# JuliaParallel/DistributedArrays.jl

Hardware: NVIDIA H100
Metric: GB/s for map! and sum on Float32 DArray (higher is better)
Workload: dtype f32

## Files before the change

distributedarrays.jl_b200/_broadcast.py:

```python
from __future__ import annotations

import ctypes as C
import struct
from typing import Callable, List, Optional, Sequence, Tuple

import numpy as np

from builtins import any as builtins_any

from . import _lib
from ._darray import B200Array, DArray, dab_dtype, darray, makelocal
from .layout import shape_of
from .runtime import close_remote_reads, open_remote_reads, runtime

_RANK = {"bool": 0, "i32": 1, "i64": 2, "i128": 3, "f32": 4, "f64": 5}


class _TagTypes(dict):

    def __missing__(self, tag):
        raise _lib.UnsupportedError(_lib.ERR_UNSUPPORTED, f"values of type {tag} have no array element type on the GPU backend "
                                    "(Int128 is served as the value type of mapreduce(f, op, d) only)")


_NPT = _TagTypes({"bool": np.dtype(np.bool_), "i32": np.dtype(np.int32), "i64": np.dtype(np.int64), "f32": np.dtype(np.float32),
                  "f64": np.dtype(np.float64), "c64": np.dtype(np.complex64), "c128": np.dtype(np.complex128)})
_TAG = {v: k for k, v in _NPT.items()}
SLICE_TRACING = [0]
_CT = {"bool": "bool", "i32": "int", "i64": "long long", "i128": "i128", "f32": "float", "f64": "double", "c64": "jl_c64", "c128": "jl_c128"}
_COMP = {"c64": "f32", "c128": "f64"}
_CPLX_OF = {"f32": "c64", "f64": "c128"}


def is_ctag(t: str) -> bool:
    return t in _COMP


def tag_of(dtype) -> str:
    dt = np.dtype(dtype)
    if dt not in _TAG:
        raise _lib.UnsupportedError(_lib.ERR_UNSUPPORTED, f"element type {dt} not served by the GPU backend")
    return _TAG[dt]


def promote(a: str, b: str) -> str:
    if a == b:
        return a
    if is_ctag(a) or is_ctag(b):
        if "i128" in (a, b):
            raise _lib.UnsupportedError(_lib.ERR_UNSUPPORTED, "Int128 values mixed with complex values are not served")
        return _CPLX_OF[promote(_COMP.get(a, a), _COMP.get(b, b))]
    if "f" in a[0] + b[0]:
        fl = [t for t in (a, b) if t[0] == "f"]
        return "f64" if "f64" in fl else "f32"
    return a if _RANK[a] >= _RANK[b] else b

# ... 706 lines not shown


def _localise(rt, a, I, pid) -> LocalArg:
    if isinstance(a, DArray):
        view = _bcview(a.dims, I)
        arr = makelocal(a, view, pid)
        return LocalArg(arr, None, tag_of(a.dtype), temp=arr is not a.chunks.get(pid))
    if isinstance(a, np.ndarray) and a.ndim > 0:
        view = _bcview(a.shape, I)
        sl = a[tuple(slice(lo - 1, hi) for lo, hi in view)]
        return LocalArg(B200Array.from_numpy(rt, sl), None, tag_of(a.dtype), temp=True)
    e = Expr.wrap(a.item() if isinstance(a, np.ndarray) else a)
    return LocalArg(None, e.val, e.jt)


def _remote_args(dest_layout, args) -> List[DArray]:
    return [a for a in args if isinstance(a, DArray) and not (a.layout.pids == dest_layout.pids and a.layout.indices == dest_layout.indices)]


def _broadcast_chunks(dest: DArray, expr: Expr, args) -> DArray:
    rt = dest.rt
    fenced = open_remote_reads(rt, _remote_args(dest.layout, args), "host")
    for pid, out in dest.chunks.items():
        I = dest.layout.localindices(pid)
        largs = [_localise(rt, a, I, pid) for a in args]
        run_local(rt, expr, out, largs)
        for la in largs:
            if la.temp and la.arr is not None:
                la.arr.free()
    close_remote_reads(rt, fenced, "host")
    return dest


def _materialise_views(args):
    from ._darray import SubDArray
    out, temps = [], []
    for a in args:
        if isinstance(a, SubDArray):
            a = a.to_darray()
            temps.append(a)
        out.append(a)
    return out, temps


def broadcast_into(dest: DArray, f: Callable, *args) -> DArray:
    args, _views = _materialise_views(args)
    try:
        return _broadcast_into(dest, f, *args)
    finally:
        for v in _views:
            v.close()


def _broadcast_into(dest: DArray, f: Callable, *args) -> DArray:
    shapes = [a.dims if isinstance(a, DArray) else (a.shape if isinstance(a, np.ndarray) else ()) for a in args]
    for shp in shapes:
        for k, s in enumerate(shp):
            want = dest.dims[k] if k < len(dest.dims) else 1
            if s != 1 and s != want:
                raise _lib.DimensionMismatch(_lib.ERR_DIM_MISMATCH, f"destination axes {dest.dims} are not compatible with source axes {tuple(shp)}")
    expr = trace(f, [_arg_tag(a) for a in args])
    return _broadcast_chunks(dest, expr, args)


def broadcast(f: Callable, *args, rt=None) -> DArray:
    args, _views = _materialise_views(args)
    try:
        return _broadcast(f, *args, rt=rt)
    finally:
        for v in _views:
            v.close()


def _broadcast(f: Callable, *args, rt=None) -> DArray:
    rt = rt or next((a.rt for a in args if isinstance(a, DArray)), None) or runtime()
    shapes = [a.dims if isinstance(a, DArray) else (a.shape if isinstance(a, np.ndarray) else ()) for a in args]
    dims = _bc_shape(shapes)
    expr = trace(f, [_arg_tag(a) for a in args])
    out_dt = _NPT[expr.jt]
    dest = darray(lambda I: B200Array.empty(rt, shape_of(I), out_dt), dims, dtype=out_dt, rt=rt)
    return _broadcast_chunks(dest, expr, args)


def copy(d: DArray) -> DArray:
    from ._darray import similar
    return _broadcast_into(similar(d), lambda x: x, d)


deepcopy = copy


def drandn(dims, procs=None, dist=None, dtype=np.float64, seed: int = 1234, rt=None) -> DArray:
    from ._darray import component_dtype, drand
    dt = np.dtype(dtype)
    if dt.kind == "c":
        ct = component_dtype(dt)
        re = drandn(dims, procs, dist, dtype=ct, seed=seed, rt=rt)
        im = drandn(dims, procs, dist, dtype=ct, seed=seed + 2, rt=rt)
        from ._darray import darray_like
        out = darray_like(lambda I: B200Array.empty(re.rt, shape_of(I), dt), re, dtype=dt)
        _broadcast_into(out, lambda a, b: complex_(0.7071067811865476 * a, 0.7071067811865476 * b), re, im)
        re.close()
        im.close()
        return out
    if dt.kind != "f":
        raise _lib.UnsupportedError(_lib.ERR_UNSUPPORTED, f"drandn of eltype {dt}")
    u1 = drand(dims, procs, dist, dtype=dt, seed=seed, rt=rt)
    u2 = drand(dims, procs, dist, dtype=dt, seed=seed + 1, rt=rt)
# ... 48 lines not shown
```

distributedarrays.jl_b200/_darray.py:

```python
from __future__ import annotations

import ctypes as C
import itertools
import weakref
from typing import Callable, Dict, List, Optional, Sequence, Tuple

import numpy as np

from . import _lib
from .layout import Layout, Range, default_procs, layout_from_chunk_shapes, make_layout, rlen, shape_of, slab_plan
from .runtime import Runtime, close_remote_reads, open_remote_reads, runtime

_DT = {np.dtype(np.float32): _lib.F32, np.dtype(np.float64): _lib.F64, np.dtype(np.int32): _lib.I32,
       np.dtype(np.int64): _lib.I64, np.dtype(np.bool_): _lib.U8,
       np.dtype(np.complex64): _lib.C64, np.dtype(np.complex128): _lib.C128}
_NP = {_lib.F32: np.dtype(np.float32), _lib.F64: np.dtype(np.float64), _lib.I32: np.dtype(np.int32),
       _lib.I64: np.dtype(np.int64), _lib.U8: np.dtype(np.bool_), _lib.C64: np.dtype(np.complex64), _lib.C128: np.dtype(np.complex128)}


def dab_dtype(dt) -> int:
    dt = np.dtype(dt)
    if dt not in _DT:
        raise _lib.UnsupportedError(_lib.ERR_UNSUPPORTED, f"element type {dt} is not served by the GPU backend (no host fallback)")
    return _DT[dt]


def np_dtype(code: int) -> np.dtype:
    return _NP[code]


def is_complex(dt) -> bool:
    return np.dtype(dt).kind == "c"


def component_dtype(dt) -> np.dtype:
    dt = np.dtype(dt)
    return {np.dtype(np.complex64): np.dtype(np.float32), np.dtype(np.complex128): np.dtype(np.float64)}.get(dt, dt)


_allowscalar = [True]


def allowscalar(flag: bool = True):
    _allowscalar[0] = bool(flag)


class B200Array:

    __slots__ = ("rt", "ptr", "shape", "dtype", "_own", "_keep", "_temp")

    def __init__(self, rt: Runtime, ptr: int, shape: Sequence[int], dtype, own: bool = True, keep=None, temp: bool = False):
        self.rt, self.ptr, self.shape, self.dtype = rt, int(ptr), tuple(int(s) for s in shape), np.dtype(dtype)
        self._own, self._keep, self._temp = own, keep, temp

    @classmethod
    def empty(cls, rt: Runtime, shape: Sequence[int], dtype, temp: bool = False) -> "B200Array":
        dtype = np.dtype(dtype)
        n = int(np.prod(shape)) if len(shape) else 1
        ptr = rt.alloc_temp(n * dtype.itemsize) if temp else rt.alloc(n * dtype.itemsize)
        return cls(rt, ptr, shape, dtype, temp=temp)

    @classmethod
    def from_numpy(cls, rt: Runtime, a: np.ndarray) -> "B200Array":
        a = np.asarray(a)
        dab_dtype(a.dtype)
        out = cls.empty(rt, a.shape, a.dtype)
        out.copy_from_host(a)
        return out

    @property
    def size(self) -> int:
        return int(np.prod(self.shape)) if len(self.shape) else 1

    @property
    def nbytes(self) -> int:
        return self.size * self.dtype.itemsize

    @property
    def ndim(self) -> int:
        return len(self.shape)

    def copy_from_host(self, a: np.ndarray, sync: bool = True):
        a = np.asarray(a, dtype=self.dtype)
        if tuple(a.shape) != self.shape:
            raise _lib.DimensionMismatch(_lib.ERR_DIM_MISMATCH, f"host array {a.shape} vs chunk {self.shape}")
        if self.size == 0:
            return
        if not a.flags.f_contiguous:
            if a.ndim == 2 and a.strides[0] == a.itemsize and a.strides[1] > 0:
                _lib.call("dab_h2d_2d", self.rt.ctx, C.c_void_p(self.ptr), a.shape[0] * a.itemsize, C.c_void_p(a.ctypes.data),
                          a.strides[1], a.shape[0] * a.itemsize, a.shape[1])
                if sync:
                    self.rt.sync()
                return
            a = np.asfortranarray(a)
        _lib.call("dab_h2d", self.rt.ctx, C.c_void_p(self.ptr), C.c_void_p(a.ctypes.data), self.nbytes)
        if sync:
            self.rt.sync()

    def to_numpy(self) -> np.ndarray:
        out = np.empty(self.shape, dtype=self.dtype, order="F")
        if self.size:
            _lib.call("dab_d2h", self.rt.ctx, C.c_void_p(out.ctypes.data), C.c_void_p(self.ptr), self.nbytes)
            self.rt.sync()
        return out

    def free(self):
        if self._own and self.ptr:
            if self._temp:
                self.rt.free_temp(self.ptr)
            else:
                self.rt.free(self.ptr)
        self.ptr = 0

    def __repr__(self):
        return f"B200Array({self.dtype}, {self.shape}, ptr=0x{self.ptr:x}, dev={self.rt.device})"


def pinned_empty(rt: Runtime, shape, dtype) -> np.ndarray:
    dtype = np.dtype(dtype)
    n = int(np.prod(shape)) if len(shape) else 1
    p = C.c_void_p()
    _lib.call("dab_host_alloc", rt.ctx, max(1, n * dtype.itemsize), C.byref(p))
    buf = (C.c_char * max(1, n * dtype.itemsize)).from_address(p.value)
    arr = np.frombuffer(buf, dtype=dtype, count=n).reshape(shape, order="F")
# ... 655 lines not shown
```

distributedarrays.jl_b200/_mapreduce.py:

```python
from __future__ import annotations

import builtins
import ctypes as C
import operator
from itertools import accumulate
from typing import Callable, Dict, Optional, Sequence, Tuple

import numpy as np

from . import _lib
from ._broadcast import Expr, broadcast, is_ctag, tag_of, trace, _NPT
from ._darray import B200Array, DArray, component_dtype, dab_dtype, is_complex, np_dtype
from .layout import Layout, ravel, reduction_passes, shape_of, unravel
from .runtime import close_remote_reads, deliver, exchange_stacks, open_remote_reads

_OPS = {"+": _lib.SUM, "add": _lib.SUM, "sum": _lib.SUM, "*": _lib.PROD, "mul": _lib.PROD, "prod": _lib.PROD, "max": _lib.MAX,
        "min": _lib.MIN}
_OPF = {operator.add: _lib.SUM, operator.mul: _lib.PROD, builtins.max: _lib.MAX, builtins.min: _lib.MIN, np.add: _lib.SUM,
        np.multiply: _lib.PROD, np.maximum: _lib.MAX, np.minimum: _lib.MIN}


def _op_code(op) -> int:
    if isinstance(op, str) and op in _OPS:
        return _OPS[op]
    if op in _OPF:
        return _OPF[op]
    raise _lib.UnsupportedError(_lib.ERR_UNSUPPORTED, f"reduction operator {op!r} is not served by a kernel (no host fallback)")


_CMPMAP = {"eq": _lib.MAP_EQ, "ne": _lib.MAP_NE, "lt": _lib.MAP_LT, "le": _lib.MAP_LE, "gt": _lib.MAP_GT, "ge": _lib.MAP_GE}
_FLIP = {"lt": "gt", "le": "ge", "gt": "lt", "ge": "le", "eq": "eq", "ne": "ne"}


def classify_map(f: Optional[Callable], dtype) -> Tuple[Optional[int], Optional[np.ndarray], Optional[Expr]]:
    if f is None:
        return _lib.MAP_ID, None, None
    tag = tag_of(dtype)
    e = trace(f, [tag])
    if e.op == "arg":
        return _lib.MAP_ID, None, e
    if is_ctag(tag):
        if len(e.args) == 1 and e.args[0].op == "arg":
            code = {"abs": _lib.MAP_ABS, "abs2": _lib.MAP_ABS2, "neg": _lib.MAP_NEG, "isnan": _lib.MAP_ISNAN}.get(e.op)
            if code is not None:
                return code, None, e
        return None, None, e
    if e.jt == tag and len(e.args) == 1 and e.args[0].op == "arg":
        code = {"abs": _lib.MAP_ABS, "abs2": _lib.MAP_ABS2, "neg": _lib.MAP_NEG}.get(e.op)
        if code is not None:
            return code, None, e
    if e.op == "mul" and e.jt == tag and builtins.all(a.op == "arg" for a in e.args):
        return _lib.MAP_ABS2, None, e
    if e.op in _CMPMAP:
        l, r = e.args

        def unpromote(side, const):
            if side.op == "convert" and side.args[0].op == "arg" and side.args[0].jt == tag and const.op == "const":
                c = const.val
                if tag == "f32" and const.jt == "f64" and float(np.float32(c)) == c:
                    return side.args[0], Expr("const", (), tag, c)
                if tag in ("i32", "i64") and const.jt in ("i64",) and side.jt == "i64":
                    return side.args[0], Expr("const", (), tag, c) if -2**31 <= c < 2**31 or tag == "i64" else (side, const)
            return side, const

        l, r = unpromote(l, r)
        r, l = unpromote(r, l)
        if l.op == "arg" and r.op == "const" and l.jt == tag:
            return _CMPMAP[e.op], np.asarray(r.val, dtype=np.dtype(dtype)), e
        if r.op == "arg" and l.op == "const" and r.jt == tag:
            return _CMPMAP[_FLIP[e.op]], np.asarray(l.val, dtype=np.dtype(dtype)), e
    if e.op == "isnan" and e.args[0].op == "arg":
        return _lib.MAP_ISNAN, None, e
    return None, None, e


def _result_dtype(dtype, op: int, mapc: int) -> np.dtype:
    out = C.c_int32()
    _lib.check(_lib.lib().dab_reduce_result_dtype(dab_dtype(dtype), op, mapc, C.byref(out)))
    return np.dtype(np.int64) if out.value == _lib.I64 else np_dtype(out.value)




def _gather_slots(d: DArray, launch: Callable[[int, B200Array, int], None]) -> np.ndarray:
    rt = d.rt
    wpr = rt.workers_per_rank
    slots = B200Array.empty(rt, (16 * wpr,), np.uint8, temp=True)
    try:
        for pid, ch in d.chunks.items():
            launch(pid, ch, slots.ptr + 16 * ((pid - 1) % wpr))
        if rt.world > 1:
            allslots = B200Array.empty(rt, (16 * wpr * rt.world,), np.uint8, temp=True)
            _lib.call("dab_allgather", rt.ctx, C.c_void_p(slots.ptr), C.c_void_p(allslots.ptr), 16 * wpr)
            host = allslots.to_numpy()
            allslots.free()
        else:
            host = slots.to_numpy()
    finally:
        rt.sync()
        slots.free()
    return host.view(np.uint8)


def _fold(host: np.ndarray, pids: Sequence[int], rdt: np.dtype, op: int):
    vals = np.empty(len(pids), dtype=rdt)
    for i, pid in enumerate(pids):
        vals[i] = host[16 * (pid - 1):16 * (pid - 1) + rdt.itemsize].view(rdt)[0]
    out = np.zeros(1, dtype=rdt)
    rcode = _lib.I64 if rdt == np.dtype(np.int64) else dab_dtype(rdt)
    _lib.check(_lib.lib().dab_combine_ordered(rcode, op, C.c_void_p(vals.ctypes.data), len(pids), C.c_void_p(out.ctypes.data)))
    return out[0], vals


def _int128(b: bytes) -> int:
    return int.from_bytes(b, "little", signed=True)


def wrap128(v: int) -> int:
    v &= (1 << 128) - 1
    return v - (1 << 128) if v >> 127 else v


def fold128(vals: Sequence[int], op: int) -> int:
    acc = vals[0]
    for v in vals[1:]:
        acc = wrap128(acc + v) if op == _lib.SUM else wrap128(acc * v) if op == _lib.PROD else (max(acc, v) if op == _lib.MAX else min(acc, v))
    return acc


def _check_nonempty(d: DArray, opc: int):
    if opc in (_lib.MAX, _lib.MIN):
        for pid in d.layout.pids:
# ... 45 lines not shown
        if ch.size == 0:
            return _empty_slot(rt, opc, np.dtype(np.int64) if wide else rdt, slot_ptr)
        I = d.layout.localindices(pid)
        largs = [_localise(rt, a, I, pid) for a in args]
        e, largs = split_c128_scalars(expr, largs)
        if len(largs) > 8:
            raise _lib.UnsupportedError(_lib.ERR_UNSUPPORTED, "more than 8 mapreduce arguments (a ComplexF64 scalar counts twice) are not served")
        src = codegen(e).encode()
        n = len(largs)
        dts = (C.c_int32 * n)(*[dab_dtype(NPT[la.tag]) for la in largs])
        ptrs = (C.c_void_p * n)(*[la.arr.ptr if la.arr is not None else None for la in largs])
        scal = (C.c_uint64 * n)()
        for k, la in enumerate(largs):
            if la.arr is None:
                scal[k] = int.from_bytes(np.asarray(la.scalar, dtype=NPT[la.tag]).tobytes().ljust(8, b"\0"), "little")
            elif la.temp:
                temps.append(la.arr)
        _lib.call("dab_mapreduce_expr", rt.ctx, src, val_code, opc_k, ch.size, n, dts, ptrs, scal, C.c_void_p(slot_ptr))

    try:
        host = _gather_slots(d, launch)
    finally:
        for t in temps:
            t.free()
        close_remote_reads(rt, fenced, "host")
    if wide:
        vals = [_int128(host[16 * (pid - 1):16 * pid].tobytes()) for pid in d.layout.pids]
        res = fold128(vals, opc)
        return (res, vals) if return_partials else res
    res, vals = _fold(host, d.layout.pids, rdt, opc if opc != _lib.COUNT else _lib.SUM)
    return (res, vals) if return_partials else res


def _mapreduce_all(f, op, d: DArray, return_partials: bool = False, others: Sequence = ()):
    opc = op if isinstance(op, int) else _op_code(op)
    if others:
        expr = trace(f, [tag_of(d.dtype)] + [_arg_tag_of(a) for a in others])
        return _mapreduce_expr(expr, opc, d, others, return_partials)
    mapc, param, expr = classify_map(f, d.dtype)
    if is_complex(d.dtype) and mapc is not None and not _complex_served(opc, mapc):
        if mapc == _lib.MAP_ID and opc in (_lib.MAX, _lib.MIN):
            raise TypeError(f"MethodError: no method matching isless(::{d.dtype}, ::{d.dtype}) -- complex numbers are not ordered")
        mapc = None
        if expr is None:
            expr = trace(lambda z: z, [tag_of(d.dtype)])
    if mapc is None:
        return _mapreduce_expr(expr, opc, d, (), return_partials)
    _check_nonempty(d, opc)
    rt = d.rt
    pp = C.c_void_p(param.ctypes.data) if param is not None else None
    rdt = _result_dtype(d.dtype, opc, mapc)
    if rt.workers_per_rank == 1 and d.layout.pids == rt.workers() and not return_partials:
        ch = d.chunks[rt.myid()]
        out = np.zeros(2, dtype=np.uint64)
        _lib.call("dab_mapreduce_all", rt.ctx, dab_dtype(d.dtype), opc, mapc, pp, C.c_void_p(ch.ptr), ch.size, C.c_void_p(out.ctypes.data))
        return out.view(np.uint8)[:rdt.itemsize].view(rdt)[0]
    code = dab_dtype(d.dtype)
    host = _gather_slots(d, lambda pid, ch, slot: _lib.call("dab_reduce", rt.ctx, code, opc, mapc, pp, C.c_void_p(ch.ptr), ch.size, C.c_void_p(slot)))
    res, vals = _fold(host, d.layout.pids, rdt, opc)
    return (res, vals) if return_partials else res


def _complex_served(opc: int, mapc: int) -> bool:
    out = C.c_int32()
    return _lib.lib().dab_reduce_result_dtype(_lib.C64, opc, mapc, C.byref(out)) == _lib.OK


def _arg_tag_of(a) -> str:
    from ._broadcast import _arg_tag
    return _arg_tag(a)


def reduce(op, d: DArray, dims=None, init=None):
    return mapreduce(None, op, d, dims=dims, init=init)


def mapreduce(f: Optional[Callable], op, d: DArray, *ds, dims=None, init=None, _partials: bool = False):
    from ._darray import SubDArray
    if isinstance(d, Expr):
        from . import _slices
        if _slices.tracing():
            return _slices.reduce_of_slice(f, op, d, ds, dims, init)
    if isinstance(d, SubDArray):
        tmp = d.to_darray()
        try:
            return mapreduce(f, op, tmp, *ds, dims=dims, init=init, _partials=_partials)
        finally:
            if dims is None:
                tmp.close()
    if dims is None:
        if init is not None:
            raise _lib.UnsupportedError(_lib.ERR_UNSUPPORTED, "mapreduce(f, op, d; init) without dims falls back to scalar iteration in the reference; not served")
        return _mapreduce_all(f, op, d, _partials, ds)
    if ds:
        tmp = broadcast(f, d, *ds)
        try:
            return mapreducedim(None, op, tmp, dims, init)
        finally:
            tmp.close()
    return mapreducedim(f, op, d, dims, init)


def sum(d: DArray, f: Optional[Callable] = None, dims=None):
    return mapreduce(f, "+", d, dims=dims)


def prod(d: DArray, f: Optional[Callable] = None, dims=None):
    return mapreduce(f, "*", d, dims=dims)

# ... 363 lines not shown
```

distributedarrays.jl_b200/csrc/dab_comm.cu:

```cuda
#include <dlfcn.h>
#include <nccl.h>

#include "dab_common.cuh"
#include "dab_scalar_ops.cuh"

namespace {

struct NcclApi {
    void* handle = nullptr;
    ncclResult_t (*GetUniqueId)(ncclUniqueId*) = nullptr;
    ncclResult_t (*CommInitRank)(ncclComm_t*, int, ncclUniqueId, int) = nullptr;
    ncclResult_t (*CommDestroy)(ncclComm_t) = nullptr;
    ncclResult_t (*AllGather)(const void*, void*, size_t, ncclDataType_t, ncclComm_t, cudaStream_t) = nullptr;
    ncclResult_t (*AllReduce)(const void*, void*, size_t, ncclDataType_t, ncclRedOp_t, ncclComm_t, cudaStream_t) = nullptr;
    ncclResult_t (*Send)(const void*, size_t, ncclDataType_t, int, ncclComm_t, cudaStream_t) = nullptr;
    ncclResult_t (*Recv)(void*, size_t, ncclDataType_t, int, ncclComm_t, cudaStream_t) = nullptr;
    ncclResult_t (*GroupStart)() = nullptr;
    ncclResult_t (*GroupEnd)() = nullptr;
    const char* (*GetErrorString)(ncclResult_t) = nullptr;
    const char* (*GetLastError)(ncclComm_t) = nullptr;
    bool ok = false;
    char why[256] = "";
};

NcclApi& nccl() {
    static NcclApi api;
    static bool tried = false;
    if (tried) return api;
    tried = true;
    const char* names[] = {"libnccl.so.2", "libnccl.so", nullptr};
    for (int i = 0; names[i] && !api.handle; ++i) api.handle = dlopen(names[i], RTLD_NOW | RTLD_GLOBAL);
    if (!api.handle) {
        snprintf(api.why, sizeof(api.why), "dlopen(libnccl.so.2) failed: %s", dlerror());
        return api;
    }
#define SYM(field, name)                                                            \
    do {                                                                            \
        *(void**)(&api.field) = dlsym(api.handle, name);                            \
        if (!api.field) {                                                           \
            snprintf(api.why, sizeof(api.why), "libnccl lacks symbol %s", name);    \
            return api;                                                             \
        }                                                                           \
    } while (0)
    SYM(GetUniqueId, "ncclGetUniqueId");
    SYM(CommInitRank, "ncclCommInitRank");
    SYM(CommDestroy, "ncclCommDestroy");
    SYM(AllGather, "ncclAllGather");
    SYM(AllReduce, "ncclAllReduce");
    SYM(Send, "ncclSend");
    SYM(Recv, "ncclRecv");
    SYM(GroupStart, "ncclGroupStart");
    SYM(GroupEnd, "ncclGroupEnd");
    SYM(GetErrorString, "ncclGetErrorString");
#undef SYM
// ... 109 lines not shown
}

int32_t dab_allreduce(dab_ctx* ctx, int32_t dtype, int32_t op, const void* send_dev, void* recv_dev, size_t count) {
    DAB_ENTER(ctx);
    NEED_COMM(ctx);
    ncclDataType_t dt;
    switch (dtype) {
        case DAB_F32: dt = ncclFloat32; break;
        case DAB_F64: dt = ncclFloat64; break;
        case DAB_I32: dt = ncclInt32; break;
        case DAB_I64: dt = ncclInt64; break;
        case DAB_U8: dt = ncclUint8; break;
        default: return dab_fail(ctx, DAB_ERR_ARG, "dab_allreduce: bad dtype %d", dtype);
    }
    ncclRedOp_t ro;
    switch (op) {
        case DAB_SUM: ro = ncclSum; break;
        case DAB_PROD: ro = ncclProd; break;
        case DAB_MAX: ro = ncclMax; break;
        case DAB_MIN: ro = ncclMin; break;
        default: return dab_fail(ctx, DAB_ERR_ARG, "dab_allreduce: bad op %d", op);
    }
    DAB_NCCL(ctx, api.AllReduce(send_dev, recv_dev, count, dt, ro, (ncclComm_t)ctx->comm, ctx->stream));
    ctx->launches++;
    return DAB_OK;
}

int32_t dab_group_start(dab_ctx* ctx) {
    DAB_ENTER(ctx);
    NEED_COMM(ctx);
    DAB_NCCL(ctx, api.GroupStart());
    return DAB_OK;
}
int32_t dab_group_end(dab_ctx* ctx) {
    DAB_ENTER(ctx);
    NEED_COMM(ctx);
    DAB_NCCL(ctx, api.GroupEnd());
    ctx->launches++;
    return DAB_OK;
}
int32_t dab_send(dab_ctx* ctx, const void* send_dev, size_t nbytes, int32_t peer) {
    DAB_ENTER(ctx);
    NEED_COMM(ctx);
    DAB_NCCL(ctx, api.Send(send_dev, nbytes, ncclInt8, peer, (ncclComm_t)ctx->comm, ctx->stream));
    return DAB_OK;
}
int32_t dab_recv(dab_ctx* ctx, void* recv_dev, size_t nbytes, int32_t peer) {
    DAB_ENTER(ctx);
    NEED_COMM(ctx);
    DAB_NCCL(ctx, api.Recv(recv_dev, nbytes, ncclInt8, peer, (ncclComm_t)ctx->comm, ctx->stream));
    return DAB_OK;
}

int32_t dab_mapreduce_all(dab_ctx* ctx, int32_t dtype, int32_t op, int32_t map, const void* map_param, const void* x, size_t n,
                          void* out_host) {
    DAB_ENTER_NOFLUSH(ctx);
    int32_t rdt;
    if (!out_host || op == DAB_EXTREMA || dab_reduce_result_dtype(dtype, op, map, &rdt) != DAB_OK) {
        DAB_FLUSH(ctx);
        DAB_REQUIRE(ctx, out_host, DAB_ERR_ARG, "dab_mapreduce_all: null out");
        if (op == DAB_EXTREMA) return dab_fail(ctx, DAB_ERR_UNSUPPORTED, "dab_mapreduce_all: extrema combines through dab_reduce + dab_allgather");
        return dab_fail(ctx, DAB_ERR_ARG, "bad dtype/op");
    }
    const bool cplx = rdt == DAB_C64 || rdt == DAB_C128;
    if ((ctx->mbox_ranks > 1 || !ctx->comm || ctx->nranks == 1) && n > 0 && !cplx) {
        ctx->fuse_op = op;
        int32_t st = dab_reduce(ctx, dtype, op, map, map_param, x, n, ctx->result_slot);
        ctx->fuse_op = -1;
        if (st != DAB_OK) return st;
        DAB_CUDA(ctx, cudaStreamSynchronize(ctx->stream));
        const volatile unsigned long long* h = (const volatile unsigned long long*)ctx->host_slot;
        if (h[1] != 0) return dab_fail(ctx, DAB_ERR_NCCL, "fused combine timed out waiting for a peer's chunk result (did every rank call?)");
        unsigned long long bits = h[0];
        memset(out_host, 0, 8);
        memcpy(out_host, &bits, dab_dtype_size(rdt));
        return DAB_OK;
    }
    if (cplx && ctx->mbox_ranks > 1 && !ctx->comm) {
        DAB_FLUSH(ctx);
        return dab_fail(ctx, DAB_ERR_UNSUPPORTED, "dab_mapreduce_all: a complex result across %d ranks needs the NCCL communicator "
                        "(the mailbox combine carries 8-byte results)", ctx->mbox_ranks);
    }
    int32_t st = dab_reduce(ctx, dtype, op, map, map_param, x, n, ctx->result_slot);
    if (st != DAB_OK) return st;
    const int P = ctx->comm ? ctx->nranks : 1;
    const void* src = ctx->result_slot;
    if (P > 1) {
        NEED_COMM(ctx);
        DAB_NCCL(ctx, api.AllGather(ctx->result_slot, ctx->gather_slots, 16, ncclInt8, (ncclComm_t)ctx->comm, ctx->stream));
        ctx->launches++;
        src = ctx->gather_slots;
    }
    DAB_CUDA(ctx, cudaMemcpyAsync(ctx->host_slot, src, (size_t)P * 16, cudaMemcpyDeviceToHost, ctx->stream));
    DAB_CUDA(ctx, cudaStreamSynchronize(ctx->stream));
    unsigned char tmp[DAB_MAX_RANKS * 16];
    size_t es = dab_dtype_size(rdt);
    for (int i = 0; i < P; ++i) memcpy(tmp + (size_t)i * es, (const char*)ctx->host_slot + (size_t)i * 16, es);
    unsigned char res[16] = {0};
    st = dab_combine_ordered(rdt, op, tmp, (size_t)P, res);
    if (st != DAB_OK) return dab_fail(ctx, st, "%s", dab_last_error(nullptr));
    memset(out_host, 0, es > 8 ? es : 8);
    memcpy(out_host, res, es);
    return DAB_OK;
}

int32_t dab_mailbox_create(dab_ctx* ctx, void* handle64) {
    DAB_ENTER(ctx);
    DAB_REQUIRE(ctx, handle64, DAB_ERR_ARG, "dab_mailbox_create: null handle");
    if (!ctx->mailbox) {
        DAB_CUDA(ctx, cudaMalloc(&ctx->mailbox, DAB_MBOX_BYTES));
        DAB_CUDA(ctx, cudaMemset(ctx->mailbox, 0, DAB_MBOX_BYTES));
    }
    cudaIpcMemHandle_t h;
    DAB_CUDA(ctx, cudaIpcGetMemHandle(&h, ctx->mailbox));
    memcpy(handle64, &h, 64);
    return DAB_OK;
}

int32_t dab_mailbox_attach(dab_ctx* ctx, const void* handles, int32_t rank, int32_t nranks) {
    DAB_ENTER(ctx);
    DAB_REQUIRE(ctx, handles && nranks >= 1 && nranks <= DAB_MAX_RANKS && rank >= 0 && rank < nranks, DAB_ERR_ARG, "dab_mailbox_attach: bad arguments");
    DAB_REQUIRE(ctx, ctx->mailbox, DAB_ERR_ARG, "dab_mailbox_attach: call dab_mailbox_create first");
    DAB_REQUIRE(ctx, ctx->mbox_ranks == 0, DAB_ERR_ARG, "mailboxes already attached");
// ... 107 lines not shown
```

distributedarrays.jl_b200/csrc/dab_common.cuh:

```cuda
#pragma once
#include <cuda_runtime.h>

#include <cstdint>
#include <cstdio>
#include <cstring>

#include "../../include/dab200.h"

#define DAB_MAX_REDUCE_BLOCKS 262144
#define DAB_SLOT_BYTES 64
#define DAB_MAX_RANKS 64

struct dab_pending_affine {
    int active;
    int32_t dtype;
    void* y;
    const void* x;
    size_t n;
    unsigned char a[8], b[8];
};

struct dab_ctx {
    int device;
    int sm_count;
    cudaStream_t stream;
    void* block_partials;
    unsigned int* counter;
    void* result_slot;
    void* gather_slots;
    void* host_slot;
    void* dim_scratch;
    size_t dim_scratch_bytes;
    uint64_t launches;
    void* comm;
    int rank, nranks;
    void* mailbox;
    void** peer_mbox_dev;
    void* peer_mbox_host[DAB_MAX_RANKS];
    int mbox_ranks;
    unsigned long long mbox_seq;
    unsigned long long barrier_seq;
    int fuse_op;
    struct dab_alloc_cache* cache;
    void* sort_dev;
    size_t sort_dev_bytes;
    void* stage[2];
    cudaEvent_t stage_ev[2];
    void* sort_host;
    unsigned long long sort_epoch;
    void* scan_dev;
    size_t scan_dev_bytes;
    unsigned long long scan_epoch;
    unsigned long long scan_tickets;
    void* scan_scratch;
    size_t scan_scratch_bytes;
    long long opt_combine_timeout_ms;
    int opt_ew_tma;
    dab_pending_affine pending;
    int defer_off;
    char err[512];
};

extern thread_local char dab_tls_err[512];

int32_t dab_fail(dab_ctx* ctx, int32_t status, const char* fmt, ...);
int32_t dab_fail_cuda(dab_ctx* ctx, cudaError_t e, const char* what, const char* file, int line);

#define DAB_CUDA(ctx, call)                                                             \
    do {                                                                                \
        cudaError_t e__ = (call);                                                       \
        if (e__ != cudaSuccess) return dab_fail_cuda((ctx), e__, #call, __FILE__, __LINE__); \
    } while (0)

#define DAB_REQUIRE(ctx, cond, status, ...)                          \
    do {                                                             \
        if (!(cond)) return dab_fail((ctx), (status), __VA_ARGS__);  \
    } while (0)

int32_t dab_flush_pending(dab_ctx* ctx);

#define DAB_FLUSH(ctx)                                    \
    do {                                                  \
        if ((ctx)->pending.active) {                      \
            int32_t st__ = dab_flush_pending(ctx);        \
            if (st__ != DAB_OK) return st__;              \
        }                                                 \
    } while (0)

#define DAB_ENTER(ctx)                                                      \
    do {                                                                    \
        if ((ctx) == nullptr) return dab_fail(nullptr, DAB_ERR_ARG, "null ctx"); \
        DAB_CUDA((ctx), cudaSetDevice((ctx)->device));                      \
        DAB_FLUSH(ctx);                                                     \
// ... 93 lines not shown
```

distributedarrays.jl_b200/csrc/dab_reduce.cu:

```cuda
#include <type_traits>

#include <cmath>

#include "dab_reduce_traits.cuh"

namespace {

struct NoStore {
    template <typename T>
    __device__ __forceinline__ void vec(Pack<T>&, size_t) const {}
    template <typename T>
    __device__ __forceinline__ T scalar(T v, size_t) const { return v; }
};
template <typename T>
struct AffineStore {
    AffineF<T> f;
    T* y;
    int4* yv;
    __device__ __forceinline__ void vec(Pack<T>& p, size_t i) const {
#pragma unroll
        for (int k = 0; k < Pack<T>::N; ++k) p.v[k] = f(p.v[k]);
        st_stream(yv + i, as_int4(p));
    }
    __device__ __forceinline__ T scalar(T v, size_t i) const {
// ... 45 lines not shown
                for (int w = VPT; w > 1; w >>= 1)
#pragma unroll
                    for (int k = 0; k < w / 2; ++k) m[k] = R::tile(m[k], m[k + w / 2]);
                tv[u] = m[0];
            }
#pragma unroll
            for (int w = RD_UNROLL; w > 1; w >>= 1)
#pragma unroll
                for (int k = 0; k < w / 2; ++k) tv[k] = R::tile(tv[k], tv[k + w / 2]);
            acc = R::comb(acc, R::lift(tv[0]));
        } else {
#pragma unroll
            for (int u = 0; u < RD_UNROLL; ++u) {
                Pack<T> p = as_pack<T>(r[u]);
                st.vec(p, base + (size_t)u * RD_THREADS);
                acc = fold_into<R>(acc, p, map);
            }
        }
    }
    if (blockIdx.x == gridDim.x - 1) {
        for (size_t i = ntiles * TILE + threadIdx.x; i < nvec; i += RD_THREADS) {
            Pack<T> p = as_pack<T>(ld_stream(xv + i));
            st.vec(p, i);
            W m = R::pre(map(p.v[0]));
#pragma unroll
            for (int k = 1; k < VPT; ++k) m = R::tile(m, R::pre(map(p.v[k])));
            acc = R::comb(acc, R::lift(m));
        }
        for (size_t i = threadIdx.x; i < head; i += RD_THREADS) acc = R::comb(acc, R::lift(R::pre(map(st.scalar(x[i], i)))));
        for (size_t i = head + nvec * VPT + threadIdx.x; i < n; i += RD_THREADS)
            acc = R::comb(acc, R::lift(R::pre(map(st.scalar(x[i], i)))));
    }
    acc = block_reduce<R>(acc, smem);
    A fin;
    if (!last_cta_out<R>(acc, partials, counter, smem, is_last, fin)) return;
    if (threadIdx.x == 0) {
        if constexpr (std::is_arithmetic<A>::value) {
            Out res;
            if (finalize_mode == 1) res = (Out)(fin == (A)n_for_all);
            else if (finalize_mode == 2) res = (Out)(fin != (A)0);
            else res = (Out)fin;
            memcpy(out, &res, sizeof(Out));
            if (sizeof(Out) < 8) memset((char*)out + sizeof(Out), 0, 8 - sizeof(Out));
            A wide = fin;
            memcpy((char*)out + 8, &wide, sizeof(A));
            if (sizeof(A) < 8) memset((char*)out + 8 + sizeof(A), 0, 8 - sizeof(A));
            if (fc.host_out && fc.nranks <= 1) {
                unsigned long long bits = 0;
                memcpy(&bits, &res, sizeof(Out));
                volatile unsigned long long* h = reinterpret_cast<volatile unsigned long long*>(fc.host_out);
                h[0] = bits;
                h[1] = 0ull;
                __threadfence_system();
            }
        } else if constexpr (is_cplx<Out>::value) {
            using CT = decltype(Out::re);
            const Out res{(CT)fin.re, (CT)fin.im};
            memset(out, 0, 16);
            memcpy(out, &res, sizeof(Out));
        } else {
            memset(out, 0, 16);
            memcpy(out, &fin, sizeof(A));
        }
    }
    if constexpr (!std::is_arithmetic<Out>::value) return;
    else {
    if (fc.nranks <= 1) return;
    __shared__ unsigned long long pay[2];
    __shared__ unsigned long long got[DAB_MAX_RANKS];
    __shared__ int timed_out;
    if (threadIdx.x == 0) {
        memcpy(&pay[0], out, 8);
        memcpy(&pay[1], (char*)out + 8, 8);
        timed_out = 0;
    }
    __syncthreads();
    const size_t bank = (size_t)(fc.seq & 1ull) * DAB_MAX_RANKS * DAB_MBOX_SLOT;
    if (threadIdx.x < (unsigned)fc.nranks) {
        volatile unsigned long long* dst =
            reinterpret_cast<volatile unsigned long long*>((char*)fc.peers[threadIdx.x] + bank + (size_t)fc.rank * DAB_MBOX_SLOT);
        dst[0] = pay[0];
        dst[1] = pay[1];
        __threadfence_system();
        dst[2] = fc.seq;
        volatile unsigned long long* src =
            reinterpret_cast<volatile unsigned long long*>((char*)fc.peers[fc.rank] + bank + (size_t)threadIdx.x * DAB_MBOX_SLOT);
        const unsigned long long t0 = dab_globaltimer_ns();
        unsigned int spins = 0;
        while (src[2] != fc.seq) {
            if ((++spins & 1023u) == 0 && dab_globaltimer_ns() - t0 > fc.timeout_ns) {
                timed_out = 1;
                break;
            }
        }
        __threadfence_system();
        got[threadIdx.x] = src[0];
    }
    __syncthreads();
    if (threadIdx.x == 0) {
        Out a;
        memcpy(&a, &got[0], sizeof(Out));
        for (int j = 1; j < fc.nranks; ++j) {
            Out b;
            memcpy(&b, &got[j], sizeof(Out));
            switch (fc.op) {
                case DAB_SUM: case DAB_COUNT: a = jl::add(a, b); break;
                case DAB_PROD: a = jl::mul(a, b); break;
                case DAB_MAX: a = jl::max(a, b); break;
                case DAB_MIN: a = jl::min(a, b); break;
                case DAB_ALL: a = (Out)(a != (Out)0 && b != (Out)0); break;
                default: a = (Out)(a != (Out)0 || b != (Out)0); break;
            }
        }
        unsigned long long bits = 0;
        memcpy(&bits, &a, sizeof(Out));
        volatile unsigned long long* h = reinterpret_cast<volatile unsigned long long*>(fc.host_out);
        h[0] = bits;
        h[1] = (unsigned long long)timed_out;
        __threadfence_system();
    }
    }
}

template <typename T, typename Map, typename R, typename Out, typename St = NoStore>
int32_t launch_reduce(dab_ctx* ctx, const T* x, size_t n, Map map, void* out, int finalize_mode, St st = St()) {
    const FlatGrid fg = flat_grid(x, n);
    if constexpr (!std::is_same<St, NoStore>::value) st.yv = reinterpret_cast<int4*>(st.y + fg.head);
    FusedComm fc;
    memset(&fc, 0, sizeof(fc));
    if (ctx->fuse_op >= 0 && ctx->mbox_ranks > 1) {
        fc.peers = ctx->peer_mbox_dev;
        fc.host_out = ctx->host_slot;
        fc.seq = ++ctx->mbox_seq;
        fc.timeout_ns = (unsigned long long)ctx->opt_combine_timeout_ms * 1000000ull;
        fc.rank = ctx->rank;
        fc.nranks = ctx->mbox_ranks;
        fc.op = ctx->fuse_op;
    } else if (ctx->fuse_op >= 0) {
        fc.host_out = ctx->host_slot;
        fc.nranks = 1;
        fc.op = ctx->fuse_op;
    }
    reduce_kernel<T, Map, R, Out, St><<<(unsigned)fg.grid, RD_THREADS, 0, ctx->stream>>>(
        x, n, fg.head, map, (typename R::A*)ctx->block_partials, ctx->counter, out, finalize_mode, (long long)n, fg.tiles_per_cta, fc, st);
    DAB_LAUNCHED(ctx);
    return DAB_OK;
}

template <typename T>
using ResultOfSum = typename std::conditional<std::is_floating_point<T>::value, T, long long>::type;

template <typename T, int FN>
int32_t reduce_arith(dab_ctx* ctx, int32_t op, const T* x, size_t n, void* out) {
    MapF<T, FN> map{(T)0};
    switch (op) {
        case DAB_SUM: return launch_reduce<T, MapF<T, FN>, SumTraits<T>, ResultOfSum<T>>(ctx, x, n, map, out, 0);
        case DAB_PROD: return launch_reduce<T, MapF<T, FN>, ProdTraits<T>, ResultOfSum<T>>(ctx, x, n, map, out, 0);
        case DAB_MAX: return launch_reduce<T, MapF<T, FN>, MaxTraits<T>, T>(ctx, x, n, map, out, 0);
        case DAB_MIN: return launch_reduce<T, MapF<T, FN>, MinTraits<T>, T>(ctx, x, n, map, out, 0);
        case DAB_EXTREMA:
            if constexpr (FN == DAB_MAP_ID) return launch_reduce<T, ExtMapF<T>, ExtremaTraits<T>, Pair<T>>(ctx, x, n, ExtMapF<T>{(T)0}, out, 0);
            else return dab_fail(ctx, DAB_ERR_UNSUPPORTED, "extrema with a map is not served (no host fallback)");
        default: return dab_fail(ctx, DAB_ERR_UNSUPPORTED, "reduce op %d needs a predicate map (no host fallback)", op);
    }
}

template <typename T, int FN>
int32_t reduce_pred(dab_ctx* ctx, int32_t op, const T* x, size_t n, const void* param, void* out) {
    PredF<T, FN> map{param ? *(const T*)param : (T)0};
    int mode;
    switch (op) {
        case DAB_ALL: mode = 1; break;
        case DAB_ANY: mode = 2; break;
        case DAB_COUNT:
        case DAB_SUM: mode = 0; break;
        default: return dab_fail(ctx, DAB_ERR_UNSUPPORTED, "reduce op %d on a predicate map (no host fallback)", op);
    }
    return launch_reduce<T, PredF<T, FN>, CountTraits, long long>(ctx, x, n, map, out, mode);
}

template <typename T>
int32_t reduce_t(dab_ctx* ctx, int32_t op, int32_t map, const void* param, const T* x, size_t n, void* out) {
    switch (map) {
        case DAB_MAP_ID: return reduce_arith<T, DAB_MAP_ID>(ctx, op, x, n, out);
        case DAB_MAP_ABS: return reduce_arith<T, DAB_MAP_ABS>(ctx, op, x, n, out);
        case DAB_MAP_ABS2: return reduce_arith<T, DAB_MAP_ABS2>(ctx, op, x, n, out);
        case DAB_MAP_NEG: return reduce_arith<T, DAB_MAP_NEG>(ctx, op, x, n, out);
#define P(FN) \
    case FN: return reduce_pred<T, FN>(ctx, op, x, n, param, out)
            P(DAB_MAP_EQ);
            P(DAB_MAP_NE);
            P(DAB_MAP_LT);
// ... 337 lines not shown
```

Before: 4310.

## Cache affine broadcast plans, spin-wait on fused reduce result, trim host overhead

Result: no change. 4387 (median of 6 runs) (+1.8%).

```diff
diff --git a/distributedarrays.jl_b200/_broadcast.py b/distributedarrays.jl_b200/_broadcast.py
--- a/distributedarrays.jl_b200/_broadcast.py
+++ b/distributedarrays.jl_b200/_broadcast.py
@@ -2,6 +2,7 @@
 
 import ctypes as C
 import struct
+import types
 from typing import Callable, List, Optional, Sequence, Tuple
 
 import numpy as np
@@ -814,8 +815,90 @@
             v.close()
 
 
+_AFFINE_PLANS: dict = {}
+_AFFINE_PLANS_MAX = 256
+
+
+def _pinned_value(v):
+    t = type(v)
+    if t is int or t is bool:
+        return t, v
+    if t is float:
+        return t, struct.pack("<d", v)
+    if t is complex:
+        return t, struct.pack("<dd", v.real, v.imag)
+    if isinstance(v, (np.number, np.bool_)):
+        return t, v.tobytes()
+    return None
+
+
+def _trace_key(f, tags: Tuple[str, ...]):
+    if type(f) is not types.FunctionType or f.__defaults__ or f.__kwdefaults__:
+        return None
+    code = f.__code__
+    if code.co_names or builtins_any(isinstance(c, types.CodeType) for c in code.co_consts):
+        return None
+    cells = []
+    for cell in f.__closure__ or ():
+        try:
+            p = _pinned_value(cell.cell_contents)
+        except ValueError:
+            return None
+        if p is None:
+            return None
+        cells.append(p)
+    return code, tuple(cells), tags
+
+
+def _affine_plan(f, x_tag: str, out_dtype: np.dtype):
+    key = _trace_key(f, (x_tag,))
+    if key is None:
+        return None
+    key = key + (out_dtype,)
+    if key in _AFFINE_PLANS:
+        return _AFFINE_PLANS[key]
+    expr = trace(f, [x_tag])
+    out_tag = tag_of(out_dtype)
+    plan = None
+    if (not uses_complex(expr) and not is_ctag(x_tag) and expr.jt == out_tag == x_tag and out_tag != "bool"
+            and all(_only_arg0(expr))):
+        ab = match_affine(expr)
+        if ab is not None:
+            a, b = np.asarray(ab[0], dtype=out_dtype), np.asarray(ab[1], dtype=out_dtype)
+            plan = (a, b, C.c_void_p(a.ctypes.data), C.c_void_p(b.ctypes.data))
+    if len(_AFFINE_PLANS) >= _AFFINE_PLANS_MAX:
+        _AFFINE_PLANS.clear()
+    _AFFINE_PLANS[key] = plan
+    return plan
+
+
+def _broadcast_affine(dest: DArray, f: Callable, args) -> bool:
+    if len(args) != 1:
+        return False
+    x = args[0]
+    if type(x) is not DArray or type(dest) is not DArray or x.dims != dest.dims:
+        return False
+    if x.layout is not dest.layout and (x.layout.pids != dest.layout.pids or x.layout.indices != dest.layout.indices):
+        return False
+    plan = _affine_plan(f, tag_of(x.dtype), dest.dtype)
+    if plan is None:
+        return False
+    rt = dest.rt
+    _, _, a_ptr, b_ptr = plan
+    code = dab_dtype(dest.dtype)
+    rt.last_kernel = "fixed"
+    for pid, out in dest.chunks.items():
+        n = out.size
+        if n:
+            _lib.call("dab_affine", rt.ctx, code, C.c_void_p(out.ptr), C.c_void_p(x.chunks[pid].ptr), a_ptr, b_ptr, n)
+            rt.last_kernel = "dab_affine"
+    return True
+
+
 def _broadcast_into(dest: DArray, f: Callable, *args) -> DArray:
-    shapes = [a.dims if isinstance(a, DArray) else (a.shape if isinstance(a, np.ndarray) else ()) for a in args]
+    if _broadcast_affine(dest, f, args):
+        return dest
+    shapes =[a.dims if isinstance(a, DArray) else (a.shape if isinstance(a, np.ndarray) else ()) for a in args]
     for shp in shapes:
         for k, s in enumerate(shp):
             want = dest.dims[k] if k < len(dest.dims) else 1
diff --git a/distributedarrays.jl_b200/_darray.py b/distributedarrays.jl_b200/_darray.py
--- a/distributedarrays.jl_b200/_darray.py
+++ b/distributedarrays.jl_b200/_darray.py
@@ -2,6 +2,7 @@
 
 import ctypes as C
 import itertools
+import math
 import weakref
 from typing import Callable, Dict, List, Optional, Sequence, Tuple
 
@@ -70,7 +71,7 @@
 
     @property
     def size(self) -> int:
-        return int(np.prod(self.shape)) if len(self.shape) else 1
+        return math.prod(self.shape)
 
     @property
     def nbytes(self) -> int:
diff --git a/distributedarrays.jl_b200/_mapreduce.py b/distributedarrays.jl_b200/_mapreduce.py
--- a/distributedarrays.jl_b200/_mapreduce.py
+++ b/distributedarrays.jl_b200/_mapreduce.py
@@ -75,9 +75,16 @@
 
 
 def _result_dtype(dtype, op: int, mapc: int) -> np.dtype:
-    out = C.c_int32()
-    _lib.check(_lib.lib().dab_reduce_result_dtype(dab_dtype(dtype), op, mapc, C.byref(out)))
-    return np.dtype(np.int64) if out.value == _lib.I64 else np_dtype(out.value)
+    key = (np.dtype(dtype), op, mapc)
+    rdt = _RESULT_DTYPES.get(key)
+    if rdt is None:
+        out = C.c_int32()
+        _lib.check(_lib.lib().dab_reduce_result_dtype(dab_dtype(dtype), op, mapc, C.byref(out)))
+        rdt = _RESULT_DTYPES[key] = np.dtype(np.int64) if out.value == _lib.I64 else np_dtype(out.value)
+    return rdt
+
+
+_RESULT_DTYPES: Dict[Tuple[np.dtype, int, int], np.dtype] = {}
 
 
 
@@ -229,9 +236,9 @@
     rdt = _result_dtype(d.dtype, opc, mapc)
     if rt.workers_per_rank == 1 and d.layout.pids == rt.workers() and not return_partials:
         ch = d.chunks[rt.myid()]
-        out = np.zeros(2, dtype=np.uint64)
-        _lib.call("dab_mapreduce_all", rt.ctx, dab_dtype(d.dtype), opc, mapc, pp, C.c_void_p(ch.ptr), ch.size, C.c_void_p(out.ctypes.data))
-        return out.view(np.uint8)[:rdt.itemsize].view(rdt)[0]
+        out = (C.c_uint64 * 2)()
+        _lib.call("dab_mapreduce_all", rt.ctx, dab_dtype(d.dtype), opc, mapc, pp, C.c_void_p(ch.ptr), ch.size, out)
+        return np.frombuffer(out, dtype=rdt, count=1)[0]
     code = dab_dtype(d.dtype)
     host = _gather_slots(d, lambda pid, ch, slot: _lib.call("dab_reduce", rt.ctx, code, opc, mapc, pp, C.c_void_p(ch.ptr), ch.size, C.c_void_p(slot)))
     res, vals = _fold(host, d.layout.pids, rdt, opc)
diff --git a/distributedarrays.jl_b200/csrc/dab_comm.cu b/distributedarrays.jl_b200/csrc/dab_comm.cu
--- a/distributedarrays.jl_b200/csrc/dab_comm.cu
+++ b/distributedarrays.jl_b200/csrc/dab_comm.cu
@@ -1,5 +1,7 @@
 #include <dlfcn.h>
 #include <nccl.h>
+
+#include <chrono>
 
 #include "dab_common.cuh"
 #include "dab_scalar_ops.cuh"
@@ -215,6 +217,24 @@
     return DAB_OK;
 }
 
+static cudaError_t wait_fused_scalar(dab_ctx* ctx, unsigned long long seq) {
+    constexpr std::chrono::milliseconds kFusedSpinBound{100};
+    const volatile unsigned long long* h = (const volatile unsigned long long*)ctx->host_slot;
+    const auto t0 = std::chrono::steady_clock::now();
+    for (unsigned spins = 1;; ++spins) {
+        if (h[2] == seq) return cudaSuccess;
+        if ((spins & 4095u) == 0) {
+            const cudaError_t q = cudaStreamQuery(ctx->stream);
+            if (q != cudaErrorNotReady) {
+                const cudaError_t s = cudaStreamSynchronize(ctx->stream);
+                return s != cudaSuccess ? s : q;
+            }
+            if (std::chrono::steady_clock::now() - t0 > kFusedSpinBound) break;
+        }
+    }
+    return cudaStreamSynchronize(ctx->stream);
+}
+
 int32_t dab_mapreduce_all(dab_ctx* ctx, int32_t dtype, int32_t op, int32_t map, const void* map_param, const void* x, size_t n,
                           void* out_host) {
     DAB_ENTER_NOFLUSH(ctx);
@@ -228,10 +248,12 @@
     const bool cplx = rdt == DAB_C64 || rdt == DAB_C128;
     if ((ctx->mbox_ranks > 1 || !ctx->comm || ctx->nranks == 1) && n > 0 && !cplx) {
         ctx->fuse_op = op;
+        const unsigned long long seq0 = ctx->host_seq;
         int32_t st = dab_reduce(ctx, dtype, op, map, map_param, x, n, ctx->result_slot);
         ctx->fuse_op = -1;
         if (st != DAB_OK) return st;
-        DAB_CUDA(ctx, cudaStreamSynchronize(ctx->stream));
+        if (ctx->host_seq != seq0) DAB_CUDA(ctx, wait_fused_scalar(ctx, ctx->host_seq));
+        else DAB_CUDA(ctx, cudaStreamSynchronize(ctx->stream));
         const volatile unsigned long long* h = (const volatile unsigned long long*)ctx->host_slot;
         if (h[1] != 0) return dab_fail(ctx, DAB_ERR_NCCL, "fused combine timed out waiting for a peer's chunk result (did every rank call?)");
         unsigned long long bits = h[0];
diff --git a/distributedarrays.jl_b200/csrc/dab_common.cuh b/distributedarrays.jl_b200/csrc/dab_common.cuh
--- a/distributedarrays.jl_b200/csrc/dab_common.cuh
+++ b/distributedarrays.jl_b200/csrc/dab_common.cuh
@@ -39,6 +39,7 @@
     void* peer_mbox_host[DAB_MAX_RANKS];
     int mbox_ranks;
     unsigned long long mbox_seq;
+    unsigned long long host_seq;
     unsigned long long barrier_seq;
     int fuse_op;
     struct dab_alloc_cache* cache;
diff --git a/distributedarrays.jl_b200/csrc/dab_reduce.cu b/distributedarrays.jl_b200/csrc/dab_reduce.cu
--- a/distributedarrays.jl_b200/csrc/dab_reduce.cu
+++ b/distributedarrays.jl_b200/csrc/dab_reduce.cu
@@ -121,6 +121,8 @@
                 h[0] = bits;
                 h[1] = 0ull;
                 __threadfence_system();
+                h[2] = fc.seq;
+                __threadfence_system();
             }
         } else if constexpr (is_cplx<Out>::value) {
             using CT = decltype(Out::re);
@@ -207,6 +209,7 @@
         fc.op = ctx->fuse_op;
     } else if (ctx->fuse_op >= 0) {
         fc.host_out = ctx->host_slot;
+        if constexpr (std::is_arithmetic<typename R::A>::value) fc.seq = ++ctx->host_seq;
         fc.nranks = 1;
         fc.op = ctx->fuse_op;
     }
```
